# FreditorK/Tensor-Train-Interior-Point-Method

Hardware: AMD Instinct MI355X
Metric: sec/IPM-iter (AMEn KKT solve), maxcut dim=10 r=1; MFMA util% on core-contract (lower is better)
Workload: dtype f64

## Files before the change

include/ttk.h:

```cpp
#ifndef TTK_H
#define TTK_H

#include <stdint.h>

#ifdef __cplusplus
extern "C" {
#endif

enum ttk_status {
  TTK_OK = 0,
  TTK_ERR_ARG = 1,
  TTK_ERR_HIP = 2,
  TTK_ERR_NOT_PD = 3,
  TTK_ERR_SINGULAR = 4,
  TTK_ERR_NOT_CONVERGED = 5,
  TTK_ILL_CONDITIONED = 6
};

typedef struct ttk_ctx_s *ttk_ctx;
int ttk_ctx_create(void *stream, ttk_ctx *out);
int ttk_ctx_destroy(ttk_ctx ctx);
int ttk_ctx_bind(ttk_ctx ctx);
void *ttk_ctx_stream(ttk_ctx ctx);

enum ttk_knob {
  TTK_KNOB_FUSED_APPLY = 0,
  TTK_KNOB_FUSED_MFMA = 1,
  TTK_KNOB_SPLITK = 2,
  TTK_KNOB_SPLITK_MINK = 3,
  TTK_KNOB_LGMRES_MW_MIN = 4,
  TTK_KNOB_MFMA_CSPLIT = 5,
  TTK_KNOB_APPLY_DUAL = 6,
  TTK_KNOB_RCOND_EXACT = 7,
  TTK_KNOB_SCHUR_ONE = 8,
  TTK_KNOB_ARNOLDI_ONE = 9,
  TTK_KNOB_SCHUR_PREP = 10,
  TTK_KNOB_SPLITK_FUSED = 11,
  TTK_KNOB_TRI_HOIST = 12,
  TTK_KNOB_TRI_ONE = 13,
  TTK_KNOB_TRI_PERSIST = 14,
  TTK_KNOB_SYEV_WAVES8 = 15,
  TTK_KNOB_BT_STAGE = 16,
  TTK_KNOB_COUNT = 17
};
int ttk_ctx_set_knob(ttk_ctx ctx, int knob, int value, int *old);
int ttk_ctx_get_knob(ttk_ctx ctx, int knob, int *value);

const char *ttk_last_error(void);
int ttk_version(void);
long long ttk_launch_count(void);
long long ttk_sync_count(void);

int ttk_gemm_offs(void *stream, const double *A, const double *B, double *C, const int64_t *offs,
                  int nb, int M, int N, int K, double alpha, double beta);

int ttk_gemm_offs_grouped(void *stream, const double *const *Aptr, const double *const *Bptr,
                          double *const *Cptr, const int64_t *offs, int ngroups, int nb, int M,
                          int N, int K, double alpha, double beta);
int ttk_einsum(void *stream, const char *eq, const int64_t *desc, double *out, double alpha, double beta);

int ttk_fused_set_mfma(int on);
int ttk_mfma_profile(unsigned long long *out8, int reset);
int ttk_dep_timeouts(unsigned *out, int reset);

int ttk_einsum_batch_begin(void *stream);
int ttk_einsum_batch_flush(void *stream);
int ttk_einsum_batch_end(void *stream);
int ttk_einsum_batch_stats(long long *out3);

typedef struct {
  const double *phi;
  const double *x;
  const double *A;
  const double *y;
  double *out;
  int64_t phi_shape[3], x_shape[3], A_shape[4], y_shape[3];
  int64_t a_strides[4];
} ttk_env_block;
int ttk_env_update(ttk_ctx ctx, int backward, int nblocks, const ttk_env_block *blocks);

int ttk_rank_scan_sync(void *stream, double *res, const double *negs, int64_t n, int nq, double *host_out);
int ttk_einsum_set_fused(int on);
int ttk_einsum_stats(long long *out);
int ttk_contract_timing(int on);
int ttk_contract_stats(double *out, int reset);

int ttk_gemm_set_splitk(int on);
int ttk_gemm_hist(int on, const char *dump_path);
int ttk_linalg_hist(int on, const char *dump_path);

int ttk_copy_nd(void *stream, const double *src, double *dst, int ndim, const int64_t *shape,
                const int64_t *sstride, const int64_t *dstride, double alpha, double beta);
int ttk_mul_nd(void *stream, const double *src, const double *src2, double *dst, int ndim,
               const int64_t *shape, const int64_t *sstride, const int64_t *s2stride,
               const int64_t *dstride, double alpha, double beta);
int ttk_recip(void *stream, const double *src, double *dst, int64_t n);
int ttk_copy_many(void *stream, int n, const double *const *src, double *const *dst, const int64_t *count);
int ttk_tt_join(void *stream, const double *a, const double *b, double *out, int ra, int Ra, int rb,
                int Rb, int64_t mid, int mode);
int ttk_axpby_nd(void *stream, const double *src, const double *src2, double *dst, int ndim,
                 const int64_t *shape, const int64_t *sstride, const int64_t *s2stride,
                 const int64_t *dstride, double alpha, double beta, double gamma);
int ttk_normalize(void *stream, const double *x, double *out, int ndim, const int64_t *shape,
                  const int64_t *xstride);
int ttk_scale_axis_ss(void *stream, const double *src, double *dst, int ndim, const int64_t *shape,
                      const int64_t *sstride, const int64_t *dstride, int axis, const double *ss, int invert);
int ttk_rayleigh_tail_sync(void *stream, const double *v, double *Mv, int64_t n, double *ev_out,
                           double *res2_out);
int ttk_rayleigh_tail_dev(void *stream, const double *v, double *Mv, int64_t n, double *out2);
int ttk_scale_axis(void *stream, const double *src, double *dst, int ndim, const int64_t *shape,
                   const int64_t *sstride, const int64_t *dstride, int axis, const double *scales);
int ttk_fill(void *stream, double *dst, int64_t n, double value);
int ttk_add_diag(void *stream, double *A, int n, int lda, double value);

int ttk_dot_nd_sync(void *stream, const double *x, const double *y, int ndim, const int64_t *shape,
                    const int64_t *xstride, const int64_t *ystride, double *result);
int ttk_dot_nd_dev(void *stream, const double *x, const double *y, int ndim, const int64_t *shape,
                   const int64_t *xstride, const int64_t *ystride, double *out);
int ttk_sumsq_batched(void *stream, const double *x, int64_t n, int nb, int64_t bstride, double *out);
int ttk_sumsq_batched_strided(void *stream, const double *x, int64_t n, int nb, int64_t bstride, int64_t inner,
                              int64_t ostride, double *out);
int ttk_read_sync(void *stream, const double *src, double *host_dst, int64_t n);
int ttk_upload(void *stream, const double *host, double *dev, int64_t n);

int64_t ttk_svd_work(int m, int n);
int ttk_svd(void *stream, const double *A, int m, int n, double *U, double *S, double *Vt,
// ... 142 lines not shown
```

tensor-train-interior-point-method_amd/_lib.py:

```python
import ctypes
import os

import torch

HERE = os.path.dirname(os.path.abspath(__file__))
LIB_PATH = os.environ.get("TTK_LIB_PATH") or os.path.join(HERE, "libttk.so")

if not os.path.exists(LIB_PATH):
    raise ImportError(f"libttk.so not found at {LIB_PATH}: run `python __graft_entry__.py build` "
                      "(hipcc --offload-arch=gfx950); the MI355X path has no CPU fallback")

lib = ctypes.CDLL(LIB_PATH)

c_dp = ctypes.POINTER(ctypes.c_double)
c_i64p = ctypes.POINTER(ctypes.c_int64)
c_ip = ctypes.POINTER(ctypes.c_int)
vp = ctypes.c_void_p
i32 = ctypes.c_int
i64 = ctypes.c_int64
f64 = ctypes.c_double

_SIGS = {
    "ttk_last_error": (ctypes.c_char_p, []),
    "ttk_version": (i32, []),
# ... 46 lines not shown
    "ttk_einsum_batch_stats": (i32, [vp]),
    "ttk_rank_scan_sync": (i32, [vp, vp, vp, i64, i32, vp]),
    "ttk_ctx_create": (i32, [vp, vp]),
    "ttk_ctx_destroy": (i32, [vp]),
    "ttk_ctx_bind": (i32, [vp]),
    "ttk_ctx_stream": (vp, [vp]),
    "ttk_lgmres": (i32, [vp, i64, vp, vp, i64, i32, i32, f64, i32, i32, vp]),
    "ttk_env_update": (i32, [vp, i32, i32, vp]),
    "ttk_round": (i32, [vp, i32, vp, vp, vp, f64, i32, vp]),
    "ttk_zipup": (i32, [vp, i32, i32, vp, vp, vp, vp, vp, f64, vp, vp]),
    "ttk_rand_orth_lds": (i64, [i32, vp, vp, vp]),
    "ttk_rand_orth": (i32, [vp, i32, vp, vp, vp, vp, vp, vp, vp]),
    "ttk_nystroem_lds": (i64, [i32, vp, vp, vp, vp]),
    "ttk_nystroem": (i32, [vp, i32, vp, vp, vp, vp, vp, vp, vp, vp, vp]),
    "ttk_retract_lds": (i64, [i32, vp, vp, vp]),
    "ttk_retract": (i32, [vp, i32, vp, vp, vp, vp, vp, vp]),
    "ttk_round_one_lds": (i64, [i32, vp, vp, vp]),
    "ttk_round_one": (i32, [vp, i32, vp, vp, vp, f64, i32, vp, vp]),
    "ttk_sum_round_one_lds": (i64, [i32, vp, i32, vp, vp, vp]),
    "ttk_sum_round_one": (i32, [vp, i32, vp, vp, i32, vp, f64, i32, vp, vp]),
    "ttk_prod_round_one_lds": (i64, [i32, i32, vp, vp, vp, vp, vp]),
    "ttk_prod_round_one": (i32, [vp, i32, i32, vp, vp, vp, vp, vp, f64, i32, vp, vp]),
    "ttk_affine_round_one_lds": (i64, [i32, vp, i32, vp, vp, vp]),
    "ttk_affine_round_one": (i32, [vp, i32, vp, vp, i32, vp, f64, i32, vp, vp]),
    "ttk_affine_round_many_lds": (i64, [i32, vp, vp, vp]),
    "ttk_affine_round_many": (i32, [vp, i32, vp, vp]),
    "ttk_split_kick_lds": (i64, [i32, i32, i32, i32, i32, i32, vp]),
    "ttk_split_kick": (i32, [vp, i32, i32, i32, i32, i32, i32, vp, vp, vp, vp, vp, vp]),
    "ttk_trunc_kick_lds": (i64, [i32, i32, i32, i32, i32, vp]),
    "ttk_trunc_kick": (i32, [vp, i32, i32, i32, i32, i32, f64, i32, vp, vp, vp, vp, vp]),
    "ttk_trunc_kick_read": (i32, [vp, i32, i32, i32, i32, i32, f64, i32, vp, vp, vp, vp, vp]),
    "ttk_dense_schur_solve": (i32, [vp, i64, i64, i64, vp, vp, vp, vp, vp]),
    "ttk_dense_schur_solve_ineq": (i32, [vp, i64, i64, i64, vp, vp, vp, vp]),
    "ttk_fused_set_mfma": (i32, [i32]),
    "ttk_mfma_profile": (i32, [vp, i32]),
    "ttk_dep_timeouts": (i32, [vp, i32]),
    "ttk_einsum_set_fused": (i32, [i32]),
    "ttk_qr_set_big_threshold": (i32, [i32]),
    "ttk_contract_timing": (i32, [i32]),
    "ttk_gemm_hist": (i32, [i32, ctypes.c_char_p]),
    "ttk_linalg_hist": (i32, [i32, ctypes.c_char_p]),
    "ttk_gemm_set_splitk": (i32, [i32]),
    "ttk_contract_stats": (i32, [vp, i32]),
    "ttk_syev_extreme": (i32, [vp, vp, i32, i32, vp, vp, vp]),
    "ttk_copy_many": (i32, [vp, i32, vp, vp, vp]),
    "ttk_lgmres_arnoldi_sync": (i32, [vp, vp, i32, i32, vp, i32, f64, c_dp, c_ip]),
    "ttk_schur_build": (i32, [vp, i32, i64, c_i64p, vp, c_i64p]),
    "ttk_schur_apply": (i32, [vp, i64, vp, vp]),
    "ttk_schur_free": (i32, [vp, i64]),
    "ttk_ctx_set_knob": (i32, [vp, i32, i32, c_ip]),
    "ttk_ctx_get_knob": (i32, [vp, i32, c_ip]),
    "ttk_lgmres_arnoldi_async": (i32, [vp, vp, i32, i32, vp, i32, f64, f64, f64, vp, i32, f64]),
    "ttk_lgmres_chunk": (i32, [vp, i64, vp, i32, i32, i32, vp, i32, f64, f64, f64, vp, f64]),
    "ttk_lgmres_build": (i32, [vp, vp, i32, i32, ctypes.POINTER(vp), i32, i32, vp, vp]),
    "ttk_lgmres_aug": (i32, [vp, vp, i32, i32, vp, i32, f64, vp, vp, vp]),
    "ttk_lgmres_set_mw_threshold": (i32, [i32]),
}

BLOCKING = frozenset(n for n in _SIGS if "sync" in n) | frozenset((
    "ttk_lgmres", "ttk_round", "ttk_zipup", "ttk_svd_tol_read", "ttk_dense_schur_solve", "ttk_dense_schur_solve_ineq",
    "ttk_lgmres_chunk", "ttk_lgmres_build", "ttk_lgmres_aug", "ttk_schur_build", "ttk_schur_free",
    "ttk_ctx_create", "ttk_ctx_destroy", "ttk_upload", "ttk_dep_timeouts", "ttk_debug_counters",
    "ttk_mfma_profile", "ttk_contract_stats", "ttk_gemm_hist", "ttk_linalg_hist"))
_held = ctypes.PyDLL(LIB_PATH) if os.environ.get("TTK_HOLD_GIL", "1") == "1" else None
lib_release = ctypes.CDLL(LIB_PATH) if _held is not None else lib

for _name, (_res, _args) in _SIGS.items():
    if os.environ.get("TTK_LIB_PATH") and not hasattr(lib, _name):
        continue
    _f = getattr(_held if _held is not None and _name not in BLOCKING else lib, _name)
    _f.restype = _res
    _f.argtypes = _args
    if _held is not None and _name not in BLOCKING:
        setattr(lib, _name, _f)
        _g = getattr(lib_release, _name)
        _g.restype = _res
        _g.argtypes = _args

EXPORTED = tuple(_SIGS)

TTK_OK, TTK_ERR_ARG, TTK_ERR_HIP, TTK_ERR_NOT_PD, TTK_ERR_SINGULAR, TTK_ERR_NOT_CONVERGED = range(6)
(KNOB_FUSED_APPLY, KNOB_FUSED_MFMA, KNOB_SPLITK, KNOB_SPLITK_MINK, KNOB_LGMRES_MW_MIN, KNOB_MFMA_CSPLIT, KNOB_APPLY_DUAL,
 KNOB_RCOND_EXACT, KNOB_SCHUR_ONE, KNOB_ARNOLDI_ONE, KNOB_SCHUR_PREP, KNOB_SPLITK_FUSED, KNOB_TRI_HOIST,
 KNOB_TRI_ONE, KNOB_TRI_PERSIST, KNOB_SYEV_WAVES8, KNOB_BT_STAGE) = range(17)


class SumTerm(ctypes.Structure):
    _fields_ = [("cores", vp), ("ranks", vp), ("coef", f64), ("transpose", i32)]


class AffineTerm(ctypes.Structure):
    _fields_ = [("kind", i32), ("transpose", i32), ("coef", f64), ("a", vp), ("a_ranks", vp), ("b", vp),
                ("b_ranks", vp), ("modes", vp)]


class AffineJob(ctypes.Structure):
    _fields_ = [("d", i32), ("inner", vp), ("rows", vp), ("nterms", i32), ("terms", vp), ("eps", f64), ("mode", i32),
                ("out", vp)]


class TTKError(RuntimeError):
    pass


class LinAlgError(ValueError):
    """Raised where LAPACK/SciPy would raise scipy.linalg.LinAlgError (potrf/getrf failure)."""


class LinAlgWarning(RuntimeWarning):
    """Raised (as an exception, like the reference's warnings-as-errors, src/tt_ipm.py:16) where
    scipy.linalg.solve would warn about an ill-conditioned matrix."""


def check(status, what=""):
    if status == TTK_OK:
        return
    msg = lib.ttk_last_error().decode(errors="replace")
    if status == TTK_ERR_NOT_PD:
        raise LinAlgError(msg)
    if status == TTK_ERR_SINGULAR:
        raise LinAlgError(msg)
    raise TTKError(f"{what}: status {status}: {msg}")
```

tensor-train-interior-point-method_amd/csrc/ttk_dense.hip:

```cpp
#include <hip/hip_runtime.h>

#include "ttk_common.h"
#include "ttk_internal.h"

namespace {

constexpr int NB = 32;
constexpr int GT = 32, GK = 16;

typedef double double4_t __attribute__((ext_vector_type(4)));

template <bool TA, bool TB>
__global__ __launch_bounds__(256) void gemm_strided_kernel(const double *__restrict__ A, int lda,
                                                           const double *__restrict__ B, int ldb,
                                                           double *__restrict__ C, int ldc, int M, int N, int K,
                                                           double alpha, double beta, int lower_only) {
  const int n0 = blockIdx.x * GT, m0 = blockIdx.y * GT;
  if (lower_only && n0 > m0 + GT - 1) return;
  __shared__ double As[GK][GT + 1];
  __shared__ double Bs[GK][GT + 1];
  const int tid = threadIdx.x, lane = tid & 63, wid = tid >> 6;
  const int wr = wid >> 1, wc = wid & 1;
  const int l_mn = tid & 31, l_k = tid >> 5;
  const bool am = m0 + l_mn < M, bn = n0 + l_mn < N;
  auto ld_a = [&](int k) -> double {
    if (!am || k >= K) return 0.0;
    const int i = m0 + l_mn;
    return TA ? A[(int64_t)k * lda + i] : A[(int64_t)i * lda + k];
  };
  auto ld_b = [&](int k) -> double {
    if (!bn || k >= K) return 0.0;
    const int j = n0 + l_mn;
    return TB ? B[(int64_t)j * ldb + k] : B[(int64_t)k * ldb + j];
  };
  double ra0 = ld_a(l_k), ra1 = ld_a(l_k + 8), rb0 = ld_b(l_k), rb1 = ld_b(l_k + 8);
  double4_t acc = {0.0, 0.0, 0.0, 0.0};
  for (int k0 = 0; k0 < K; k0 += GK) {
    As[l_k][l_mn] = ra0;
    As[l_k + 8][l_mn] = ra1;
    Bs[l_k][l_mn] = rb0;
    Bs[l_k + 8][l_mn] = rb1;
    __syncthreads();
    if (k0 + GK < K) {
      ra0 = ld_a(k0 + GK + l_k);
      ra1 = ld_a(k0 + GK + l_k + 8);
      rb0 = ld_b(k0 + GK + l_k);
      rb1 = ld_b(k0 + GK + l_k + 8);
    }
#pragma unroll
    for (int s = 0; s < GK / 4; ++s) {
      const double a = As[s * 4 + (lane >> 4)][wr * 16 + (lane & 15)];
      const double b = Bs[s * 4 + (lane >> 4)][wc * 16 + (lane & 15)];
      acc = __builtin_amdgcn_mfma_f64_16x16x4f64(a, b, acc, 0, 0, 0);
    }
    __syncthreads();
  }
  const int col = n0 + wc * 16 + (lane & 15);
  if (col >= N) return;
#pragma unroll
  for (int r = 0; r < 4; ++r) {
    const int row = m0 + wr * 16 + (lane >> 4) + 4 * r;
    if (row < M) {
      double *p = C + (int64_t)row * ldc + col;
      *p = beta * (*p) + alpha * acc[r];
    }
  }
}

__global__ __launch_bounds__(256) void potf2_block_kernel(double *A, int n, int k0, int kb, int *status) {
  __shared__ double Ls[NB][NB + 1];
  __shared__ int s_fail;
  const int tid = threadIdx.x;
  if (*status) return;
  ttk::staged_copy<4>(kb * kb, tid, 256, [&](int e) { return A[(int64_t)(k0 + e / kb) * n + k0 + e % kb]; },
                      [&](int e, double v) { Ls[e / kb][e % kb] = v; });
  if (tid == 0) s_fail = 0;
  __syncthreads();
  for (int j = 0; j < kb; ++j) {
    if (tid == 0) {
      const double d = Ls[j][j];
      if (!(d > 0.0)) {
        s_fail = k0 + j + 1;
      } else {
        Ls[j][j] = sqrt(d);
      }
    }
    __syncthreads();
    if (s_fail) break;
    const double inv = 1.0 / Ls[j][j];
    for (int i = j + 1 + tid; i < kb; i += 256) Ls[i][j] *= inv;
    __syncthreads();
    const int t = kb - j - 1;
    for (int e = tid; e < t * t; e += 256) {
      const int i = j + 1 + e / t, c = j + 1 + e % t;
      if (c <= i) Ls[i][c] -= Ls[i][j] * Ls[c][j];
    }
    __syncthreads();
  }
  if (s_fail) {
    if (tid == 0) *status = s_fail;
    return;
  }
  for (int e = tid; e < kb * kb; e += 256) {
    const int i = e / kb, j = e - i * kb;
    if (j <= i) A[(int64_t)(k0 + i) * n + k0 + j] = Ls[i][j];
  }
}

__global__ __launch_bounds__(256) void panel_trsm_kernel(double *A, int n, int k0, int kb, const int *status) {
  __shared__ double Ls[NB][NB + 1];
  if (*status) return;
  const int tid = threadIdx.x;
  ttk::staged_copy<4>(kb * kb, tid, 256, [&](int e) { return A[(int64_t)(k0 + e / kb) * n + k0 + e % kb]; },
                      [&](int e, double v) { Ls[e / kb][e % kb] = v; });
  __syncthreads();
  const int r = k0 + kb + blockIdx.x * 256 + tid;
  if (r >= n) return;
  double *a = A + (int64_t)r * n + k0;
  double x[NB];
#pragma unroll
  for (int j = 0; j < NB; ++j) x[j] = j < kb ? a[j] : 0.0;
#pragma unroll
  for (int j = 0; j < NB; ++j) {
    if (j < kb) {
      double s = x[j];
#pragma unroll
      for (int c = 0; c < NB; ++c)
        if (c < j) s -= x[c] * Ls[j][c];
      x[j] = s / Ls[j][j];
    }
  }
#pragma unroll
  for (int j = 0; j < NB; ++j)
    if (j < kb) a[j] = x[j];
}

__global__ __launch_bounds__(256) void zero_upper_kernel(double *A, int n, const int *status) {
  if (*status) return;
  const int64_t e = blockIdx.x * (int64_t)256 + threadIdx.x;
  if (e >= (int64_t)n * n) return;
  const int i = (int)(e / n), c = (int)(e % n);
  if (c > i) A[e] = 0.0;
}

__global__ __launch_bounds__(256) void trsm_diag_kernel(const double *__restrict__ L, int n, double *B, int nrhs,
                                                        int ldb, int r0, int kb, int trans) {
  __shared__ double Ls[NB][NB + 1];
  const int tid = threadIdx.x;
  ttk::staged_copy<4>(
      kb * kb, tid, 256,
      [&](int e) {
        const int i = e / kb, j = e - i * kb;
        return trans ? L[(int64_t)(r0 + j) * n + r0 + i] : L[(int64_t)(r0 + i) * n + r0 + j];
      },
      [&](int e, double v) { Ls[e / kb][e % kb] = v; });
  __syncthreads();
  const int c = blockIdx.x * 256 + tid;
  if (c >= nrhs) return;
  double x[NB];
#pragma unroll
  for (int j = 0; j < NB; ++j) x[j] = j < kb ? B[(int64_t)(r0 + j) * ldb + c] : 0.0;
  if (!trans) {
#pragma unroll
    for (int j = 0; j < NB; ++j) {
      if (j < kb) {
        double s = x[j];
#pragma unroll
        for (int q = 0; q < NB; ++q)
          if (q < j) s -= Ls[j][q] * x[q];
        x[j] = s / Ls[j][j];
      }
    }
  } else {
#pragma unroll
    for (int jj = NB - 1; jj >= 0; --jj) {
      if (jj < kb) {
        double s = x[jj];
#pragma unroll
        for (int q = 0; q < NB; ++q)
          if (q > jj && q < kb) s -= Ls[jj][q] * x[q];
        x[jj] = s / Ls[jj][jj];
      }
    }
  }
#pragma unroll
  for (int j = 0; j < NB; ++j)
    if (j < kb) B[(int64_t)(r0 + j) * ldb + c] = x[j];
}



__global__ __launch_bounds__(256) void colsum_kernel(const double *__restrict__ A, int n, double *__restrict__ out) {
  const int c = blockIdx.x * 256 + threadIdx.x;
  if (c >= n) return;
  out[c] = ttk::sum_ahead<8>(n, [&](int r) { return fabs(A[(int64_t)r * n + c]); }, 0.0);
}

__device__ __forceinline__ void panel_row_update(double *__restrict__ pi, const double *__restrict__ prow, int c,
                                                 int kb, double inv) {
  const double l = pi[c] * inv;
  pi[c] = l;
#pragma unroll 8
  for (int cc = c + 1; cc < kb; ++cc) pi[cc] -= l * prow[cc];
}

__global__ __launch_bounds__(1024) void getf2_panel_kernel(double *A, int n, int k0, int kb, int *piv, int *status) {
  __shared__ double wv[16];
  __shared__ int wi[16];
  __shared__ int s_p;
  const int tid = threadIdx.x, lane = tid & 63, wid = tid >> 6;
  for (int c = 0; c < kb; ++c) {
    const int j = k0 + c;
    double best = -1.0;
    int bi = j;
    for (int i = j + tid; i < n; i += 1024) {
      const double v = fabs(A[(int64_t)i * n + j]);
      if (v > best) {
        best = v;
        bi = i;
      }
    }
    ttk::wave_argmax(best, bi);
    if (lane == 0) {
      wv[wid] = best;
      wi[wid] = bi;
    }
    __syncthreads();
    if (tid == 0) {
      double b = wv[0];
      int p = wi[0];
      for (int w = 1; w < 16; ++w)
        if (wv[w] > b || (wv[w] == b && wi[w] < p)) {
          b = wv[w];
          p = wi[w];
        }
      s_p = p;
      piv[j] = p;
    }
    __syncthreads();
    const int p = s_p;
    if (p != j && tid < kb) {
      double *a = A + (int64_t)j * n + k0 + tid, *b = A + (int64_t)p * n + k0 + tid;
      const double t = *a;
      *a = *b;
      *b = t;
    }
    __syncthreads();
    const double d = A[(int64_t)j * n + j];
    if (d == 0.0) {
      if (tid == 0 && *status == 0) *status = j + 1;
      continue;
    }
    const double inv = 1.0 / d;
    const double *prow = A + (int64_t)j * n + k0;
    for (int i = j + 1 + tid; i < n; i += 1024) panel_row_update(A + (int64_t)i * n + k0, prow, c, kb, inv);
    __syncthreads();
  }
}

__global__ __launch_bounds__(1024) void getf2_panel_lds_kernel(double *A, int n, int k0, int kb, int *piv,
                                                               int *status) {
  extern __shared__ double P[];
  __shared__ double wv[16];
  __shared__ int wi[16];
  __shared__ int s_p;
  const int tid = threadIdx.x, lane = tid & 63, wid = tid >> 6, nt = blockDim.x, nw = nt >> 6;
  const int rows = n - k0, ld = kb + 1;
  ttk::staged_copy<8>(rows * kb, tid, nt, [&](int e) { return A[(int64_t)(k0 + e / kb) * n + k0 + e % kb]; },
                      [&](int e, double v) { P[(e / kb) * ld + e % kb] = v; });
  __syncthreads();
  for (int c = 0; c < kb; ++c) {
    double best = -1.0;
// ... 614 lines not shown
      dim3 grid((rest + GT - 1) / GT, (rest + GT - 1) / GT);
      hipLaunchKernelGGL((gemm_strided_kernel<false, false>), grid, dim3(256), 0, st,
                         A + (int64_t)(k0 + kb) * n + k0, n, A + (int64_t)k0 * n + k0 + kb, n,
                         A + (int64_t)(k0 + kb) * n + k0 + kb, n, rest, rest, kb, -1.0, 1.0, 0);
    }
    TTK_LAUNCH_CHECK();
    k0 += kb;
  }
  if (want_rcond == 1) return lu_rcond_launch(st, A, n, piv, colsum, status, rcond);
  return TTK_OK;
}

int lu_rcond_launch(hipStream_t st, const double *LU, int n, const int *piv, const double *colsum, const int *status,
                    double *rcond) {
  const size_t shm_perm = 3 * (size_t)n * sizeof(double) + 2 * (size_t)n * sizeof(int);
  const int use_perm = shm_perm <= 140000;
  const size_t shm = use_perm ? shm_perm : 2 * (size_t)n * sizeof(double) + (size_t)n * sizeof(int);
  if (shm > 65536)
    (void)hipFuncSetAttribute(reinterpret_cast<const void *>(lu_rcond_kernel),
                              hipFuncAttributeMaxDynamicSharedMemorySize, (int)shm);
  const int exact = ttk::ctx().knob[TTK_KNOB_RCOND_EXACT] != 0;
  hipLaunchKernelGGL(lu_rcond_kernel, dim3(1), dim3(1024), shm, st, LU, n, piv, colsum, status, rcond, use_perm,
                     exact);
  TTK_LAUNCH_CHECK();
  return TTK_OK;
}

int lu_solve_cols(hipStream_t st, const double *LU, int n, const int *piv, double *B, int nrhs, int ldb) {
  const size_t shm = (size_t)n * (sizeof(double) + sizeof(int));
  if (shm > 65536)
    (void)hipFuncSetAttribute(reinterpret_cast<const void *>(lu_solve_cols_kernel),
                              hipFuncAttributeMaxDynamicSharedMemorySize, (int)shm);
  hipLaunchKernelGGL(lu_solve_cols_kernel, dim3(nrhs), dim3(1024), shm, st, LU, n, piv, B, ldb);
  TTK_LAUNCH_CHECK();
  return TTK_OK;
}


int cholesky_blocked(hipStream_t st, double *A, int n, int *status) {
  TTK_HIP(hipMemsetAsync(status, 0, sizeof(int), st));
  for (int k0 = 0; k0 < n; k0 += NB) {
    const int kb = n - k0 < NB ? n - k0 : NB;
    hipLaunchKernelGGL(potf2_block_kernel, dim3(1), dim3(256), 0, st, A, n, k0, kb, status);
    const int rest = n - k0 - kb;
    if (rest > 0) {
      hipLaunchKernelGGL(panel_trsm_kernel, dim3((rest + 255) / 256), dim3(256), 0, st, A, n, k0, kb, status);
      double *L21 = A + (int64_t)(k0 + kb) * n + k0;
      double *A22 = A + (int64_t)(k0 + kb) * n + k0 + kb;
      dim3 grid((rest + GT - 1) / GT, (rest + GT - 1) / GT);
      hipLaunchKernelGGL((gemm_strided_kernel<false, true>), grid, dim3(256), 0, st, L21, n, L21, n, A22, n, rest,
                         rest, kb, -1.0, 1.0, 1);
    }
    TTK_LAUNCH_CHECK();
  }
  hipLaunchKernelGGL(zero_upper_kernel, dim3((unsigned)(((int64_t)n * n + 255) / 256)), dim3(256), 0, st, A, n,
                     status);
  TTK_LAUNCH_CHECK();
  return TTK_OK;
}

int trsm_blocked(hipStream_t st, const double *L, int n, double *B, int nrhs, int ldb, int trans) {
  for (int s = 0; s < n; s += NB) {
    const int kb = n - s < NB ? n - s : NB;
    const int r0 = trans ? n - s - kb : s;
    hipLaunchKernelGGL(trsm_diag_kernel, dim3((nrhs + 255) / 256), dim3(256), 0, st, L, n, B, nrhs, ldb, r0, kb,
                       trans);
    const int rest = n - s - kb;
    if (rest > 0) {
      dim3 grid((nrhs + GT - 1) / GT, (rest + GT - 1) / GT);
      if (!trans) {
        hipLaunchKernelGGL((gemm_strided_kernel<false, false>), grid, dim3(256), 0, st,
                           L + (int64_t)(r0 + kb) * n + r0, n, B + (int64_t)r0 * ldb, ldb,
                           B + (int64_t)(r0 + kb) * ldb, ldb, rest, nrhs, kb, -1.0, 1.0, 0);
      } else {
        hipLaunchKernelGGL((gemm_strided_kernel<true, false>), grid, dim3(256), 0, st, L + (int64_t)r0 * n, n,
                           B + (int64_t)r0 * ldb, ldb, B, ldb, rest, nrhs, kb, -1.0, 1.0, 0);
      }
    }
    TTK_LAUNCH_CHECK();
  }
  return TTK_OK;
}

}
```

tensor-train-interior-point-method_amd/csrc/ttk_internal.h:

```cpp
#ifndef TTK_INTERNAL_H
#define TTK_INTERNAL_H

#include <hip/hip_runtime.h>

#include <cstdlib>

#include "../../include/ttk.h"

namespace ttk {
inline int env_int(const char *name, int dflt) {
  const char *v = std::getenv(name);
  return v ? std::atoi(v) : dflt;
}
struct UpSlot {
  double *p = nullptr;
  size_t n = 0;
  hipEvent_t ev = nullptr;
  bool pending = false;
};
constexpr int UP_SLOTS = 64;

struct Ctx {
  hipStream_t stream = nullptr;
  double *scratch = nullptr;
  int64_t scratch_n = 0;
  void *batch = nullptr;
  double *splitk = nullptr;
  int64_t splitk_n = 0;
  double *dev_scalar = nullptr;
  void *schur = nullptr;
  double *schur_w = nullptr;
  int64_t schur_wcap = 0;
  unsigned *dep = nullptr;
  unsigned dep_total = 0;
  unsigned tick_total = 0;
  unsigned *splitk_cnt = nullptr;
  double *lgmres = nullptr;
  int64_t lgmres_n = 0;
  int *status = nullptr;
  double *rcond = nullptr;
  double *mapped_h = nullptr, *mapped_d = nullptr;
  size_t mapped_n = 0;
  UpSlot up[UP_SLOTS];
  int up_next = 0;
  hipStream_t side = nullptr;
  hipEvent_t ev_fork = nullptr, ev_join = nullptr;
  int knob[TTK_KNOB_COUNT] = {env_int("TTK_FUSED_APPLY", 1) != 0 ? 1 : 0, env_int("TTK_FUSED_MFMA", 1) != 0 ? 1 : 0,
                              env_int("TTK_SPLITK", 1) != 0 ? 1 : 0,
                              env_int("TTK_SPLITK_MINK", 128) > 0 ? env_int("TTK_SPLITK_MINK", 128) : 128,
                              env_int("TTK_LGMRES_MW_MIN", 16384), env_int("TTK_MFMA_CSPLIT", 1) != 0 ? 1 : 0,
                              env_int("TTK_APPLY_DUAL", 1) != 0 ? 1 : 0, env_int("TTK_RCOND_EXACT", 0) != 0 ? 1 : 0,
                              env_int("TTK_SCHUR_ONE", 1) != 0 ? 1 : 0, env_int("TTK_ARNOLDI_ONE", 0) != 0 ? 1 : 0,
                              env_int("TTK_SCHUR_PREP", 1) != 0 ? 1 : 0, env_int("TTK_SPLITK_FUSED", 1) != 0 ? 1 : 0,
                              env_int("TTK_TRI_HOIST", 1) != 0 ? 1 : 0, env_int("TTK_TRI_ONE", 0),
                              env_int("TTK_TRI_PERSIST", 0) != 0 ? 1 : 0, env_int("TTK_SYEV_WAVES8", 1) != 0 ? 1 : 0,
                              env_int("TTK_BT_STAGE", 1) != 0 ? 1 : 0};
};
Ctx &ctx();
Ctx *ctx_swap(Ctx *c);
void schur_release(Ctx &c);
int presize_splitk();
int presize_lgmres();
int presize_schur();
}

struct ttk_ctx_s {
  ttk::Ctx c;
};

namespace ttk {
struct CtxScope {
  Ctx *prev;
  bool on;
  explicit CtxScope(ttk_ctx_s *h) : prev(nullptr), on(h != nullptr) {
    if (on) prev = ctx_swap(&h->c);
  }
  ~CtxScope() {
    if (on) ctx_swap(prev);
  }
};
void ctx_free_einsum(Ctx &c);

int cholesky_blocked(hipStream_t st, double *A, int n, int *status);
int trsm_blocked(hipStream_t st, const double *L, int n, double *B, int nrhs, int ldb, int trans);
int lu_blocked(hipStream_t st, double *A, int n, int *piv, double *work, int *status, double *rcond, int want_rcond);
int lu_rcond_launch(hipStream_t st, const double *LU, int n, const int *piv, const double *colsum, const int *status,
                    double *rcond);
int lu_factor_fork_rcond(hipStream_t st, double *A, int n, int *piv, double *work, int *forked);
int lu_rcond_join(hipStream_t st);
int lu_solve_cols(hipStream_t st, const double *LU, int n, const int *piv, double *B, int nrhs, int ldb);
int qr_colmajor(void *stream, const double *At, int m, int n, double *Qt, double *R, double *work);

struct GemmProblem {
  const double *A, *B;
  double *C;
  const int64_t *offs;
  int nb, M, N, K;
  double alpha, beta;
};
bool gemm_groupable(int nb, int M, int N, int K);
int gemm_group(hipStream_t st, const GemmProblem *p, int n);
int batch_barrier(void *stream);
int upload_ring(hipStream_t st, const double *host, double *dev, int64_t n);
int schur_apply(void *stream, int64_t handle, const double *v, double *out);
}

#endif
```

tensor-train-interior-point-method_amd/csrc/ttk_linalg.hip:

```cpp
#include <math.h>
#include <stdlib.h>

#include <array>
#include <chrono>
#include <cstdio>
#include <cstring>
#include <map>
#include <mutex>

#include "ttk_common.h"
#include "ttk_internal.h"

namespace {

constexpr double EPS = 2.220446049250313e-16;
__device__ unsigned long long g_dbg[8];

constexpr int LDS_DOUBLES = 20000;

__device__ __forceinline__ void rr_pair(int P, int r, int k, int &p, int &q) {
  const int P1 = P - 1;
  if (k == 0) {
    p = r;
    q = P1;
// ... 2844 lines not shown
  }
#define TTK_SVD_WG(GG)                                                                                      \
  case GG:                                                                                                  \
    if (wmode == 2) TTK_SVD_WG_MODE(GG, 2) else TTK_SVD_WG_MODE(GG, 0)                                       \
    break;
#define TTK_SVD_WG3(GG)                                                                                     \
  case GG:                                                                                                  \
    if (wmode == 2) TTK_SVD_WG_MODE(GG, 2) else if (wmode == 1) TTK_SVD_WG_MODE(GG, 1) else TTK_SVD_WG_MODE(GG, 0) \
    break;
  switch (g) {
    TTK_SVD_WG(1)
    TTK_SVD_WG(2)
    TTK_SVD_WG3(4)
    TTK_SVD_WG3(8)
    TTK_SVD_WG3(16)
    TTK_SVD_WG(32)
    default:
      TTK_SVD_WG(64)
  }
#undef TTK_SVD_WG
#undef TTK_SVD_WG3
#undef TTK_SVD_WG_MODE
  TTK_LAUNCH_CHECK();
  return TTK_OK;
}

static const int g_qr_narrow = getenv("TTK_QR_NARROW") ? atoi(getenv("TTK_QR_NARROW")) : 1;
static int g_qr_big_k = 48;

int ttk_qr_set_big_threshold(int k) {
  const int old = g_qr_big_k;
  if (k > 0) g_qr_big_k = k;
  return old;
}

int64_t ttk_qr_work(int m, int n) {
  const int64_t k = m < n ? m : n;
  const int64_t small = (int64_t)m * n + k + (int64_t)m * k + 16, big = qr_big_work(m, n);
  return small > big ? small : big;
}

static int qr_impl(void *stream, const double *A, int m, int n, double *Q, double *R, double *work,
                   int colmajor);

int ttk_qr(void *stream, const double *A, int m, int n, double *Q, double *R, double *work) {
  return qr_impl(stream, A, m, n, Q, R, work, 0);
}

}
namespace ttk {
int qr_colmajor(void *stream, const double *At, int m, int n, double *Qt, double *R, double *work) {
  return qr_impl(stream, At, m, n, Qt, R, work, 1);
}
}
extern "C" {

static int qr_impl(void *stream, const double *A, int m, int n, double *Q, double *R, double *work,
                   int colmajor) {
  if (int brc = ttk::batch_barrier(stream)) return brc;
  if (m <= 0 || n <= 0) {
    ttk::set_error("ttk_qr: empty matrix %dx%d", m, n);
    return TTK_ERR_ARG;
  }
  const int64_t k = m < n ? m : n;
  const int64_t need = (int64_t)m * n + k + (int64_t)m * k + 16;
  const int use_lds = need <= LDS_DOUBLES;
  if (colmajor && k >= g_qr_big_k && (!use_lds || g_qr_big_k <= 2)) return TTK_ERR_ARG;
  LinalgScope scope_(TTK_STREAM(stream), 1, m, n, k >= g_qr_big_k && (!use_lds || g_qr_big_k <= 2) ? 0 : use_lds ? 1 : 2);
  if (k >= g_qr_big_k && (!use_lds || g_qr_big_k <= 2)) return qr_big(stream, A, m, n, Q, R, work);
  const size_t shm = use_lds ? need * sizeof(double) : 0;
  const int nt = (g_qr_narrow && m <= 65) ? 64 * (n < 16 ? (n < 1 ? 1 : n) : 16) : 1024;
  if (use_lds) {
    allow_big_lds(qr_kernel<true>, shm);
    hipLaunchKernelGGL(qr_kernel<true>, dim3(1), dim3(nt), shm, TTK_STREAM(stream), A, m, n, Q, R, work, use_lds, colmajor);
  } else {
    allow_big_lds(qr_kernel<false>, shm);
    hipLaunchKernelGGL(qr_kernel<false>, dim3(1), dim3(nt), shm, TTK_STREAM(stream), A, m, n, Q, R, work, use_lds, colmajor);
  }
  TTK_LAUNCH_CHECK();
  return TTK_OK;
}

static int g_dense_block_min = 96;
static int g_lu_block_min = getenv("TTK_LU_BLOCK_MIN") ? atoi(getenv("TTK_LU_BLOCK_MIN")) : 32;

int ttk_dense_set_block_min(int n) {
  const int old = g_dense_block_min;
  g_dense_block_min = n;
  return old;
}

int ttk_cholesky_sync(void *stream, double *A, int n) {
  if (int brc = ttk::batch_barrier(stream)) return brc;
  if (ensure_status()) {
    ttk::set_error("ttk_cholesky_sync: status alloc failed");
    return TTK_ERR_HIP;
  }
  LinalgScope scope_(TTK_STREAM(stream), 4, n, n, n >= g_dense_block_min);
  if (n >= g_dense_block_min) {
    const int rc = ttk::cholesky_blocked(TTK_STREAM(stream), A, n, ttk::ctx().status);
    if (rc) return rc;
  } else {
    hipLaunchKernelGGL(chol_kernel, dim3(1), dim3(1024), 0, TTK_STREAM(stream), A, n, ttk::ctx().status);
    TTK_LAUNCH_CHECK();
  }
  int st = 0;
  TTK_HIP(hipMemcpyAsync(&st, ttk::ctx().status, sizeof(int), hipMemcpyDeviceToHost, TTK_STREAM(stream)));
  ttk::note_sync();
  TTK_HIP(hipStreamSynchronize(TTK_STREAM(stream)));
  if (st) {
    ttk::set_error("%d-th leading minor of the array is not positive definite", st);
    return TTK_ERR_NOT_PD;
  }
  return TTK_OK;
}

int ttk_trsm_lower(void *stream, const double *L, int n, double *B, int nrhs, int ldb, int trans) {
  if (int brc = ttk::batch_barrier(stream)) return brc;
  if (n <= 0 || nrhs <= 0) return TTK_OK;
  if (n >= g_dense_block_min) return ttk::trsm_blocked(TTK_STREAM(stream), L, n, B, nrhs, ldb, trans);
  hipLaunchKernelGGL(trsm_kernel, dim3((nrhs + 63) / 64), dim3(256), 0, TTK_STREAM(stream), L, n, B, nrhs, ldb, trans);
  TTK_LAUNCH_CHECK();
  return TTK_OK;
}

int ttk_lu_sync(void *stream, double *A, int n, int *piv, double *work, double *rcond_out) {
  if (int brc = ttk::batch_barrier(stream)) return brc;
  if (ensure_status()) {
    ttk::set_error("ttk_lu_sync: status alloc failed");
    return TTK_ERR_HIP;
  }
  LinalgScope scope_(TTK_STREAM(stream), 3, n, n, n >= g_lu_block_min && n <= 7000);
  if (n >= g_lu_block_min && n <= 7000) {
    const int rc = ttk::lu_blocked(TTK_STREAM(stream), A, n, piv, work, ttk::ctx().status, ttk::ctx().rcond, 1);
    if (rc) return rc;
  } else {
    hipLaunchKernelGGL(lu_kernel, dim3(1), dim3(1024), 0, TTK_STREAM(stream), A, n, piv, work, ttk::ctx().status, ttk::ctx().rcond);
    TTK_LAUNCH_CHECK();
  }
  int st = 0;
  TTK_HIP(hipMemcpyAsync(&st, ttk::ctx().status, sizeof(int), hipMemcpyDeviceToHost, TTK_STREAM(stream)));
  TTK_HIP(hipMemcpyAsync(rcond_out, ttk::ctx().rcond, sizeof(double), hipMemcpyDeviceToHost, TTK_STREAM(stream)));
  ttk::note_sync();
  TTK_HIP(hipStreamSynchronize(TTK_STREAM(stream)));
  if (st) {
    ttk::set_error("Matrix is singular (zero pivot at %d).", st);
    return TTK_ERR_SINGULAR;
  }
  return TTK_OK;
}

}

namespace ttk {
int lu_factor_fork_rcond(hipStream_t st, double *A, int n, int *piv, double *work, int *forked) {
  *forked = 0;
  if (ensure_status()) {
    set_error("lu_factor_fork_rcond: status alloc failed");
    return TTK_ERR_HIP;
  }
  Ctx &c = ctx();
  LinalgScope scope_(st, 3, n, n, n >= g_lu_block_min && n <= 7000 ? 2 : 3);
  if (!(n >= g_lu_block_min && n <= 7000)) {
    hipLaunchKernelGGL(lu_kernel, dim3(1), dim3(1024), 0, st, A, n, piv, work, c.status, c.rcond);
    TTK_LAUNCH_CHECK();
    return TTK_OK;
  }
  static const int fork_on = getenv("TTK_LU_FORK") ? atoi(getenv("TTK_LU_FORK")) : 1;
  if (!fork_on) {
    const int rc = lu_blocked(st, A, n, piv, work, c.status, c.rcond, 1);
    return rc;
  }
  if (!c.side) {
    TTK_HIP(hipStreamCreateWithFlags(&c.side, hipStreamNonBlocking));
    TTK_HIP(hipEventCreateWithFlags(&c.ev_fork, hipEventDisableTiming));
    TTK_HIP(hipEventCreateWithFlags(&c.ev_join, hipEventDisableTiming));
  }
  const int rc = lu_blocked(st, A, n, piv, work, c.status, c.rcond, 2);
  if (rc) return rc;
  TTK_HIP(hipEventRecord(c.ev_fork, st));
  TTK_HIP(hipStreamWaitEvent(c.side, c.ev_fork, 0));
  const int rr = lu_rcond_launch(c.side, A, n, piv, work, c.status, c.rcond);
  if (rr) return rr;
  TTK_HIP(hipEventRecord(c.ev_join, c.side));
  *forked = 1;
  return TTK_OK;
}

int lu_rcond_join(hipStream_t st) {
  TTK_HIP(hipStreamWaitEvent(st, ctx().ev_join, 0));
  return TTK_OK;
}
}

extern "C" {

int ttk_lu_solve(void *stream, const double *LU, int n, const int *piv, double *B, int nrhs, int ldb) {
  if (int brc = ttk::batch_barrier(stream)) return brc;
  if (n >= g_lu_block_min && n <= 12000 && nrhs <= 8 && nrhs > 0) return ttk::lu_solve_cols(TTK_STREAM(stream), LU, n, piv, B, nrhs, ldb);
  if (n <= 0 || nrhs <= 0) return TTK_OK;
  hipLaunchKernelGGL(lu_solve_kernel, dim3((nrhs + 63) / 64), dim3(256), 0, TTK_STREAM(stream), LU, n, piv, B, nrhs, ldb);
  TTK_LAUNCH_CHECK();
  return TTK_OK;
// ... 158 lines not shown
```

Before: 0.08309.

## Add single-launch column-blocked TRSM kernel fusing diagonal solves and trailing updates

Adds a trsm_cols kernel where each block owns a 32-column strip of the right-hand sides and walks all diagonal blocks itself. It solves the diagonal block, then applies the trailing MFMA GEMM update across two thread groups, prefetching the next diagonal tile and the next GEMM tile into registers. This replaces the multi-launch blocked TRSM (per-step diag and GEMM kernels) for mid-size n (96..288), aiming to cut launch overhead and keep data on-chip. The GEMM kernel is refactored into reusable fetch/finish helpers with two-stage prefetch. The trade-off is limited parallelism (one block per 32 columns) and a serial diagonal solve run by only 32 threads.

New measurement: 0.08351. No clear change (+0.5%).

```diff
diff --git a/include/ttk.h b/include/ttk.h
--- a/include/ttk.h
+++ b/include/ttk.h
@@ -41,7 +41,8 @@
   TTK_KNOB_TRI_PERSIST = 14,
   TTK_KNOB_SYEV_WAVES8 = 15,
   TTK_KNOB_BT_STAGE = 16,
-  TTK_KNOB_COUNT = 17
+  TTK_KNOB_TRSM_COLS = 17,
+  TTK_KNOB_COUNT = 18
 };
 int ttk_ctx_set_knob(ttk_ctx ctx, int knob, int value, int *old);
 int ttk_ctx_get_knob(ttk_ctx ctx, int knob, int *value);
diff --git a/tensor-train-interior-point-method_amd/_lib.py b/tensor-train-interior-point-method_amd/_lib.py
--- a/tensor-train-interior-point-method_amd/_lib.py
+++ b/tensor-train-interior-point-method_amd/_lib.py
@@ -152,7 +152,7 @@
 TTK_OK, TTK_ERR_ARG, TTK_ERR_HIP, TTK_ERR_NOT_PD, TTK_ERR_SINGULAR, TTK_ERR_NOT_CONVERGED = range(6)
 (KNOB_FUSED_APPLY, KNOB_FUSED_MFMA, KNOB_SPLITK, KNOB_SPLITK_MINK, KNOB_LGMRES_MW_MIN, KNOB_MFMA_CSPLIT, KNOB_APPLY_DUAL,
  KNOB_RCOND_EXACT, KNOB_SCHUR_ONE, KNOB_ARNOLDI_ONE, KNOB_SCHUR_PREP, KNOB_SPLITK_FUSED, KNOB_TRI_HOIST,
- KNOB_TRI_ONE, KNOB_TRI_PERSIST, KNOB_SYEV_WAVES8, KNOB_BT_STAGE) = range(17)
+ KNOB_TRI_ONE, KNOB_TRI_PERSIST, KNOB_SYEV_WAVES8, KNOB_BT_STAGE, KNOB_TRSM_COLS) = range(18)
 
 
 class SumTerm(ctypes.Structure):
diff --git a/tensor-train-interior-point-method_amd/csrc/ttk_dense.hip b/tensor-train-interior-point-method_amd/csrc/ttk_dense.hip
--- a/tensor-train-interior-point-method_amd/csrc/ttk_dense.hip
+++ b/tensor-train-interior-point-method_amd/csrc/ttk_dense.hip
@@ -9,6 +9,79 @@
 constexpr int GT = 32, GK = 16;
 
 typedef double double4_t __attribute__((ext_vector_type(4)));
+
+struct TileRegs {
+  double a[4], b[4];
+  double c[4];
+};
+
+template <bool TA, bool TB>
+struct TileView {
+  const double *A, *B;
+  double *C;
+  int lda, ldb, ldc, M, N, K, m0, n0, tid;
+  __device__ __forceinline__ double ld_a(int k) const {
+    const int i = m0 + (tid & 31);
+    if (i >= M || k >= K) return 0.0;
+    return TA ? A[(int64_t)k * lda + i] : A[(int64_t)i * lda + k];
+  }
+  __device__ __forceinline__ double ld_b(int k) const {
+    const int j = n0 + (tid & 31);
+    if (j >= N || k >= K) return 0.0;
+    return TB ? B[(int64_t)j * ldb + k] : B[(int64_t)k * ldb + j];
+  }
+  __device__ __forceinline__ int col() const { return n0 + ((tid >> 6) & 1) * 16 + (tid & 15); }
+  __device__ __forceinline__ int row(int r) const { return m0 + (tid >> 7) * 16 + ((tid & 63) >> 4) + 4 * r; }
+};
+
+template <bool TA, bool TB>
+__device__ __forceinline__ TileRegs gemm_tile_fetch(const TileView<TA, TB> &v) {
+  const int l_k = v.tid >> 5;
+  TileRegs t;
+#pragma unroll
+  for (int q = 0; q < 4; ++q) {
+    t.a[q] = v.ld_a(l_k + 8 * q);
+    t.b[q] = v.ld_b(l_k + 8 * q);
+  }
+#pragma unroll
+  for (int r = 0; r < 4; ++r) t.c[r] = (v.col() < v.N && v.row(r) < v.M) ? v.C[(int64_t)v.row(r) * v.ldc + v.col()] : 0.0;
+  return t;
+}
+
+template <bool TA, bool TB>
+__device__ __forceinline__ void gemm_tile_finish(const TileView<TA, TB> &v, TileRegs t, double alpha, double beta,
+                                                 double (*As)[GT + 1], double (*Bs)[GT + 1]) {
+  const int tid = v.tid, lane = tid & 63, wid = tid >> 6;
+  const int wr = wid >> 1, wc = wid & 1;
+  const int l_mn = tid & 31, l_k = tid >> 5;
+  double4_t acc = {0.0, 0.0, 0.0, 0.0};
+  for (int k0 = 0; k0 < v.K; k0 += GK) {
+    As[l_k][l_mn] = t.a[0];
+    As[l_k + 8][l_mn] = t.a[1];
+    Bs[l_k][l_mn] = t.b[0];
+    Bs[l_k + 8][l_mn] = t.b[1];
+    __syncthreads();
+    t.a[0] = t.a[2];
+    t.a[1] = t.a[3];
+    t.b[0] = t.b[2];
+    t.b[1] = t.b[3];
+    t.a[2] = v.ld_a(k0 + 2 * GK + l_k);
+    t.a[3] = v.ld_a(k0 + 2 * GK + l_k + 8);
+    t.b[2] = v.ld_b(k0 + 2 * GK + l_k);
+    t.b[3] = v.ld_b(k0 + 2 * GK + l_k + 8);
+#pragma unroll
+    for (int s = 0; s < GK / 4; ++s) {
+      const double a = As[s * 4 + (lane >> 4)][wr * 16 + (lane & 15)];
+      const double b = Bs[s * 4 + (lane >> 4)][wc * 16 + (lane & 15)];
+      acc = __builtin_amdgcn_mfma_f64_16x16x4f64(a, b, acc, 0, 0, 0);
+    }
+    __syncthreads();
+  }
+  if (v.col() >= v.N) return;
+#pragma unroll
+  for (int r = 0; r < 4; ++r)
+    if (v.row(r) < v.M) v.C[(int64_t)v.row(r) * v.ldc + v.col()] = beta * t.c[r] + alpha * acc[r];
+}
 
 template <bool TA, bool TB>
 __global__ __launch_bounds__(256) void gemm_strided_kernel(const double *__restrict__ A, int lda,
@@ -19,52 +92,8 @@
   if (lower_only && n0 > m0 + GT - 1) return;
   __shared__ double As[GK][GT + 1];
   __shared__ double Bs[GK][GT + 1];
-  const int tid = threadIdx.x, lane = tid & 63, wid = tid >> 6;
-  const int wr = wid >> 1, wc = wid & 1;
-  const int l_mn = tid & 31, l_k = tid >> 5;
-  const bool am = m0 + l_mn < M, bn = n0 + l_mn < N;
-  auto ld_a = [&](int k) -> double {
-    if (!am || k >= K) return 0.0;
-    const int i = m0 + l_mn;
-    return TA ? A[(int64_t)k * lda + i] : A[(int64_t)i * lda + k];
-  };
-  auto ld_b = [&](int k) -> double {
-    if (!bn || k >= K) return 0.0;
-    const int j = n0 + l_mn;
-    return TB ? B[(int64_t)j * ldb + k] : B[(int64_t)k * ldb + j];
-  };
-  double ra0 = ld_a(l_k), ra1 = ld_a(l_k + 8), rb0 = ld_b(l_k), rb1 = ld_b(l_k + 8);
-  double4_t acc = {0.0, 0.0, 0.0, 0.0};
-  for (int k0 = 0; k0 < K; k0 += GK) {
-    As[l_k][l_mn] = ra0;
-    As[l_k + 8][l_mn] = ra1;
-    Bs[l_k][l_mn] = rb0;
-    Bs[l_k + 8][l_mn] = rb1;
-    __syncthreads();
-    if (k0 + GK < K) {
-      ra0 = ld_a(k0 + GK + l_k);
-      ra1 = ld_a(k0 + GK + l_k + 8);
-      rb0 = ld_b(k0 + GK + l_k);
-      rb1 = ld_b(k0 + GK + l_k + 8);
-    }
-#pragma unroll
-    for (int s = 0; s < GK / 4; ++s) {
-      const double a = As[s * 4 + (lane >> 4)][wr * 16 + (lane & 15)];
-      const double b = Bs[s * 4 + (lane >> 4)][wc * 16 + (lane & 15)];
-      acc = __builtin_amdgcn_mfma_f64_16x16x4f64(a, b, acc, 0, 0, 0);
-    }
-    __syncthreads();
-  }
-  const int col = n0 + wc * 16 + (lane & 15);
-  if (col >= N) return;
-#pragma unroll
-  for (int r = 0; r < 4; ++r) {
-    const int row = m0 + wr * 16 + (lane >> 4) + 4 * r;
-    if (row < M) {
-      double *p = C + (int64_t)row * ldc + col;
-      *p = beta * (*p) + alpha * acc[r];
-    }
-  }
+  const TileView<TA, TB> v{A, B, C, lda, ldb, ldc, M, N, K, m0, n0, (int)threadIdx.x};
+  gemm_tile_finish(v, gemm_tile_fetch(v), alpha, beta, As, Bs);
 }
 
 __global__ __launch_bounds__(256) void potf2_block_kernel(double *A, int n, int k0, int kb, int *status) {
@@ -143,20 +172,19 @@
   if (c > i) A[e] = 0.0;
 }
 
-__global__ __launch_bounds__(256) void trsm_diag_kernel(const double *__restrict__ L, int n, double *B, int nrhs,
-                                                        int ldb, int r0, int kb, int trans) {
-  __shared__ double Ls[NB][NB + 1];
-  const int tid = threadIdx.x;
+__device__ __forceinline__ void trsm_diag_stage(const double *__restrict__ L, int n, int r0, int kb, int trans,
+                                                double (*Ls)[NB + 1], int tid, int nt) {
   ttk::staged_copy<4>(
-      kb * kb, tid, 256,
+      kb * kb, tid, nt,
       [&](int e) {
         const int i = e / kb, j = e - i * kb;
         return trans ? L[(int64_t)(r0 + j) * n + r0 + i] : L[(int64_t)(r0 + i) * n + r0 + j];
       },
       [&](int e, double v) { Ls[e / kb][e % kb] = v; });
-  __syncthreads();
-  const int c = blockIdx.x * 256 + tid;
-  if (c >= nrhs) return;
+}
+
+__device__ __forceinline__ void trsm_diag_col(const double (*Ls)[NB + 1], double *B, int ldb, int r0, int kb, int trans,
+                                              int c) {
   double x[NB];
 #pragma unroll
   for (int j = 0; j < NB; ++j) x[j] = j < kb ? B[(int64_t)(r0 + j) * ldb + c] : 0.0;
@@ -188,6 +216,85 @@
     if (j < kb) B[(int64_t)(r0 + j) * ldb + c] = x[j];
 }
 
+__global__ __launch_bounds__(256) void trsm_diag_kernel(const double *__restrict__ L, int n, double *B, int nrhs,
+                                                        int ldb, int r0, int kb, int trans) {
+  __shared__ double Ls[NB][NB + 1];
+  const int tid = threadIdx.x;
+  trsm_diag_stage(L, n, r0, kb, trans, Ls, tid, 256);
+  __syncthreads();
+  const int c = blockIdx.x * 256 + tid;
+  if (c < nrhs) trsm_diag_col(Ls, B, ldb, r0, kb, trans, c);
+}
+
+#ifndef TTK_TRSM_GROUPS
+#define TTK_TRSM_GROUPS 2
+#endif
+constexpr int TRSM_GROUPS = TTK_TRSM_GROUPS, TRSM_NT = 256 * TRSM_GROUPS;
+constexpr int TRSM_PRE = (NB * NB + TRSM_NT - 1) / TRSM_NT;
+
+template <bool TA>
+__device__ __forceinline__ void trsm_update(const double *A, int lda, const double *X, double *C, int ldb, int rest,
+                                            int nrhs, int kb, int n0, int grp, int gtid, double (*As)[GT + 1],
+                                            double (*Bs)[GT + 1]) {
+  const int rounds = ((rest + GT - 1) / GT + TRSM_GROUPS - 1) / TRSM_GROUPS;
+  TileView<TA, false> v{A, X, C, lda, ldb, ldb, rest, nrhs, kb, grp * GT, n0, gtid};
+  TileRegs cur = gemm_tile_fetch(v);
+  for (int t = 0; t < rounds; ++t) {
+    TileView<TA, false> vn = v;
+    vn.m0 += TRSM_GROUPS * GT;
+    const TileRegs nxt = gemm_tile_fetch(vn);
+    gemm_tile_finish(v, cur, -1.0, 1.0, As, Bs);
+    v = vn;
+    cur = nxt;
+  }
+}
+
+__global__ __launch_bounds__(TRSM_NT) void trsm_cols_kernel(const double *__restrict__ L, int n, double *B, int nrhs,
+                                                            int ldb, int trans) {
+  __shared__ double Ls[NB][NB + 1];
+  __shared__ double As[TRSM_GROUPS][GK][GT + 1];
+  __shared__ double Bs[TRSM_GROUPS][GK][GT + 1];
+  const int tid = threadIdx.x, grp = tid >> 8, gtid = tid & 255;
+  const int n0 = blockIdx.x * GT;
+  auto diag_elem = [&](int r0, int kb, int e) -> double {
+    if (e >= kb * kb) return 0.0;
+    const int i = e / kb, j = e - i * kb;
+    return trans ? L[(int64_t)(r0 + j) * n + r0 + i] : L[(int64_t)(r0 + i) * n + r0 + j];
+  };
+  double pre[TRSM_PRE];
+  {
+    const int kb = n < NB ? n : NB;
+#pragma unroll
+    for (int u = 0; u < TRSM_PRE; ++u) pre[u] = diag_elem(trans ? n - kb : 0, kb, tid + u * TRSM_NT);
+  }
+  for (int s = 0; s < n; s += NB) {
+    const int kb = n - s < NB ? n - s : NB;
+    const int r0 = trans ? n - s - kb : s;
+#pragma unroll
+    for (int u = 0; u < TRSM_PRE; ++u) {
+      const int e = tid + u * TRSM_NT;
+      if (e < kb * kb) Ls[e / kb][e % kb] = pre[u];
+    }
+    __syncthreads();
+    if (tid < GT && n0 + tid < nrhs) trsm_diag_col(Ls, B, ldb, r0, kb, trans, n0 + tid);
+    const int rest = n - s - kb;
+    if (rest > 0) {
+      const int kn = rest < NB ? rest : NB;
+#pragma unroll
+      for (int u = 0; u < TRSM_PRE; ++u) pre[u] = diag_elem(trans ? r0 - kn : r0 + kb, kn, tid + u * TRSM_NT);
+    }
+    __threadfence_block();
+    __syncthreads();
+    if (!trans)
+      trsm_update<false>(L + (int64_t)(r0 + kb) * n + r0, n, B + (int64_t)r0 * ldb, B + (int64_t)(r0 + kb) * ldb, ldb,
+                         rest, nrhs, kb, n0, grp, gtid, As[grp], Bs[grp]);
+    else
+      trsm_update<true>(L + (int64_t)r0 * n, n, B + (int64_t)r0 * ldb, B, ldb, rest, nrhs, kb, n0, grp, gtid, As[grp],
+                        Bs[grp]);
+    __threadfence_block();
+    __syncthreads();
+  }
+}
 
 
 __global__ __launch_bounds__(256) void colsum_kernel(const double *__restrict__ A, int n, double *__restrict__ out) {
@@ -968,4 +1075,11 @@
   return TTK_OK;
 }
 
-}
+int trsm_cols(hipStream_t st, const double *L, int n, double *B, int nrhs, int ldb, int trans) {
+  hipLaunchKernelGGL(trsm_cols_kernel, dim3((nrhs + GT - 1) / GT), dim3(256 * TRSM_GROUPS), 0, st, L, n, B, nrhs, ldb,
+                     trans);
+  TTK_LAUNCH_CHECK();
+  return TTK_OK;
+}
+
+}
diff --git a/tensor-train-interior-point-method_amd/csrc/ttk_internal.h b/tensor-train-interior-point-method_amd/csrc/ttk_internal.h
--- a/tensor-train-interior-point-method_amd/csrc/ttk_internal.h
+++ b/tensor-train-interior-point-method_amd/csrc/ttk_internal.h
@@ -54,7 +54,7 @@
                               env_int("TTK_SCHUR_PREP", 1) != 0 ? 1 : 0, env_int("TTK_SPLITK_FUSED", 1) != 0 ? 1 : 0,
                               env_int("TTK_TRI_HOIST", 1) != 0 ? 1 : 0, env_int("TTK_TRI_ONE", 0),
                               env_int("TTK_TRI_PERSIST", 0) != 0 ? 1 : 0, env_int("TTK_SYEV_WAVES8", 1) != 0 ? 1 : 0,
-                              env_int("TTK_BT_STAGE", 1) != 0 ? 1 : 0};
+                              env_int("TTK_BT_STAGE", 1) != 0 ? 1 : 0, env_int("TTK_TRSM_COLS", 1)};
 };
 Ctx &ctx();
 Ctx *ctx_swap(Ctx *c);
@@ -83,6 +83,7 @@
 
 int cholesky_blocked(hipStream_t st, double *A, int n, int *status);
 int trsm_blocked(hipStream_t st, const double *L, int n, double *B, int nrhs, int ldb, int trans);
+int trsm_cols(hipStream_t st, const double *L, int n, double *B, int nrhs, int ldb, int trans);
 int lu_blocked(hipStream_t st, double *A, int n, int *piv, double *work, int *status, double *rcond, int want_rcond);
 int lu_rcond_launch(hipStream_t st, const double *LU, int n, const int *piv, const double *colsum, const int *status,
                     double *rcond);
diff --git a/tensor-train-interior-point-method_amd/csrc/ttk_linalg.hip b/tensor-train-interior-point-method_amd/csrc/ttk_linalg.hip
--- a/tensor-train-interior-point-method_amd/csrc/ttk_linalg.hip
+++ b/tensor-train-interior-point-method_amd/csrc/ttk_linalg.hip
@@ -2950,6 +2950,7 @@
 }
 
 static int g_dense_block_min = 96;
+static bool trsm_cols_wins(int n, int nrhs) { return n <= 288; }
 static int g_lu_block_min = getenv("TTK_LU_BLOCK_MIN") ? atoi(getenv("TTK_LU_BLOCK_MIN")) : 32;
 
 int ttk_dense_set_block_min(int n) {
@@ -2986,7 +2987,12 @@
 int ttk_trsm_lower(void *stream, const double *L, int n, double *B, int nrhs, int ldb, int trans) {
   if (int brc = ttk::batch_barrier(stream)) return brc;
   if (n <= 0 || nrhs <= 0) return TTK_OK;
-  if (n >= g_dense_block_min) return ttk::trsm_blocked(TTK_STREAM(stream), L, n, B, nrhs, ldb, trans);
+  if (n >= g_dense_block_min) {
+    const int cols = ttk::ctx().knob[TTK_KNOB_TRSM_COLS];
+    if (cols == 2 || (cols == 1 && trsm_cols_wins(n, nrhs)))
+      return ttk::trsm_cols(TTK_STREAM(stream), L, n, B, nrhs, ldb, trans);
+    return ttk::trsm_blocked(TTK_STREAM(stream), L, n, B, nrhs, ldb, trans);
+  }
   hipLaunchKernelGGL(trsm_kernel, dim3((nrhs + 63) / 64), dim3(256), 0, TTK_STREAM(stream), L, n, B, nrhs, ldb, trans);
   TTK_LAUNCH_CHECK();
   return TTK_OK;
```
